# TariAgentBenchmark/unet-embroidery-seg

Hardware: AMD Instinct MI355X
Metric: images/sec training unet_resnet50 512×512 bf16 at 1/2/4/8 GPUs; mIoU parity (higher is better)
Workload: dtype bf16; 1 GPU; unet_resnet50 binary seg 512x512, per-GPU batch 16, lovasz_hinge + Adam; global_batch=16, image_size=512, parallelism=dp1

## Files before the change

### include/unetseg_hip.h

```cpp
#ifndef UNETSEG_HIP_H
#define UNETSEG_HIP_H

#include <stddef.h>
#include <stdint.h>

#ifdef __cplusplus
extern "C" {
#endif

const char* unetseg_last_error(void);
int unetseg_abi_version(void);
int unetseg_device_arch(char* buf, int n);


int unetseg_pack_conv_weight(int dtype, const float* w, int K, int C, int R, int S, int Cpad, void* wk, void* wt,
                             void* stream);
typedef struct UnetsegPackDesc {
  const float* w;
  void* wk;
  void* wt;
  long long start;
  int K, C, R, S, Cpad, Kld;
} UnetsegPackDesc;
int unetseg_pack_tiles(int K, int Cpad, int taps);
int unetseg_pack_conv_weights(int dtype, const void* desc, int n, long total, void* stream);
int unetseg_conv_tile_m(void);
int unetseg_conv2d_fwd_tile_m(int dtype, int c1, int ldc1, int c2, int ldc2, int n, int h, int w, int cout, int r,
                              int s, int stride, int pad);
int unetseg_conv2d_fwd(int dtype, const void* x1, int c1, int ldc1, const void* x2, int c2, int ldc2, int n, int h,
                       int w, const void* wk, int cout, int r, int s, int stride, int pad, const float* bias, int relu,
                       void* y, int ldy, float* stats, void* stream);
int unetseg_conv2d_fwd_bnrelu_in(int dtype, const void* x1, int c1, int ldc1, int n, int h, int w, const void* wk,
                                 int cout, const float* in_sc, const float* in_sh, const float* bias, int relu,
                                 void* y, int ldy, float* stats, void* stream);
int unetseg_conv2d_fwd_bnrelu_in_config(int dtype, int c1, int ldc1, int n, int h, int w, int cout);
int unetseg_conv2d_fwd_head_ok(int dtype, int ldc1, int n, int h, int w, int ldy, int head_k);
int unetseg_conv2d_fwd_head(int dtype, const void* x1, int ldc1, int n, int h, int w, const void* wk,
                            const float* bias, void* y, int ldy, int head_k, const float* head_w, const float* head_b,
                            float* logits, void* stream);
int unetseg_conv2d_fwd_mask(int dtype, const void* x1, int ldc1, int n, int h, int w, const void* wk,
                            const float* bias, void* y, int ldy, unsigned char* mbits, void* stream);
int unetseg_conv2d_wgrad_bnrelu_in(int dtype, const void* x1, int c1, int ldc1, int n, int h, int w, const void* dy,
                                   int ldy, int cout, const float* in_sc, const float* in_sh, float* ws,
                                   size_t ws_bytes, float* dw, int dw_c, int accumulate, void* stream);
int unetseg_conv2d_fwd_affine(int dtype, const void* x1, int c1, int ldc1, const void* x2, int c2, int ldc2, int n,
                              int h, int w, const void* wk, int cout, int r, int s, int stride, int pad,
                              const float* escale, const float* bias, int relu, void* y, int ldy, void* stream);
int unetseg_conv2d_fwd_config(int dtype, int c1, int ldc1, int c2, int ldc2, int n, int h, int w, int cout, int r,
                              int s, int stride, int pad, int* taps_out);
int unetseg_conv2d_dgrad_config(int dtype, int ldy, int n, int p, int q, int cout, int cin, int r, int s, int stride,
                                int pad, int ldx, int h, int w, int* cfg_out, int* taps_out);
int unetseg_conv2d_wgrad_config(int dtype, int c1, int ldc1, int c2, int ldc2, int n, int h, int w, int ldy, int cout,
                                int r, int s, int stride, int pad, int* splits_out);
int unetseg_conv2d_dgrad(int dtype, const void* dy, int ldy, int n, int p, int q, const void* wt, int cout, int cin,
                         int r, int s, int stride, int pad, void* dx, int ldx, int h, int w, int accumulate,
                         void* stream);
int unetseg_conv2d_dgrad_post(int dtype, const void* dy, int ldy, int n, int p, int q, const void* wt, int cout,
                              int cin, int r, int s, int stride, int pad, void* dx, int ldx, int h, int w, int post,
                              const void* aux, int ld_aux, const float* psc, const float* psh, const float* pmean,
                              const float* pinv, float* part, int rows, void* stream);
int unetseg_conv2d_dgrad_post_res(int dtype, const void* dy, int ldy, int n, int p, int q, const void* wt, int cout,
                                  int cin, void* dx, int ldx, const void* y1, int ld1, const float* mean1,
                                  const float* inv1, const unsigned char* mbits, const void* y2, int ld2,
                                  const float* mean2, const float* inv2, float* part, int rows, void* stream);
size_t unetseg_conv2d_wgrad_workspace(int dtype, int n, int p, int q, int cout, int cin, int r, int s);
int unetseg_conv2d_wgrad(int dtype, const void* x1, int c1, int ldc1, const void* x2, int c2, int ldc2, int n, int h,
                         int w, const void* dy, int ldy, int cout, int r, int s, int stride, int pad, float* ws,
                         size_t ws_bytes, float* dw, int dw_c, int accumulate, void* stream);
int unetseg_conv2d_wgrad_rows(int dtype, const void* x1, int c1, int ldc1, int n, int h, int w, const void* dy,
                              int ldy, int cout, int r, int s, int stride, int pad, float* ws, size_t ws_bytes,
                              float* dw, int dw_c, int accumulate, int dw_rows, void* stream);

int unetseg_pack_input_stem(const float* x, int n, int c, int h, int w, void* xp, void* stream);
int unetseg_stem_pack_weight(const float* w, int K, int C, void* wk, void* stream);
int unetseg_stem_fwd_tile_m(int n, int h, int w, int K);
int unetseg_stem_config(int n, int h, int w, int K, int* splits_out);
int unetseg_stem_fwd(const void* xp, int n, int h, int w, const void* wk, int K, void* y, int ldy, float* stats,
                     void* stream);
size_t unetseg_stem_wgrad_workspace(int n, int h, int w, int K);
int unetseg_stem_wgrad(const void* xp, int n, int h, int w, const void* dy, int ldy, int K, float* ws,
                       size_t ws_bytes, float* dw, int C, int accumulate, void* stream);
int unetseg_pack_input(int dtype, const float* x, int n, int c, int h, int w, int cpad, void* y, void* stream);


// ... 163 lines not shown
```

### unet-embroidery-seg_amd/csrc/conv.hip

```cpp
#include <cstdlib>

#include "common.h"
#include "conv_fast.h"

namespace {

constexpr int kBM = 128;

__device__ __forceinline__ int swz8(int row, int ch) { return ch ^ ((row >> 1) & 7); }
__device__ __forceinline__ int swz_tr(int row) { return ((row & 3) | ((row >> 1) & 4)) << 1; }

struct IgemmArgs {
  const void* x1;
  const void* x2;
  int c1, c2, ldc1, ldc2;
  int N, H, W;
  int hc, wc;
  int istride;
  int r0, rs, nr, dh0, dhs;
  int s0, ss, ns, dw0, dws;
  int S;
  int cin;
  const void* wt;
  long ldw;
// ... 1085 lines not shown
  if (k > 0) US_CHECK_ARG(launch_tn_multi(m, k, st) == 0, "conv2d_dgrad_post: merged launch refused");
  US_LAUNCH_CHECK("conv2d_dgrad_post");
  return 0;
}

UNETSEG_API int unetseg_conv2d_dgrad_post_res(int dtype, const void* dy, int ldy, int n, int p, int q, const void* wt,
                                              int cout, int cin, void* dx, int ldx, const void* y1, int ld1,
                                              const float* mean1, const float* inv1, const unsigned char* mbits,
                                              const void* y2, int ld2, const float* mean2, const float* inv2,
                                              float* part, int rows, void* stream) {
  if (dtype != DT_BF16 || n <= 0 || p <= 0 || q <= 0 || cout % 8 || ldy % 8 || cin % 8 || ldx < cin || ldx % 8)
    return 0;
  IgemmArgs a;
  if (!dgrad_classes(dy ? dy : kSomePtr, ldy, n, p, q, wt ? wt : kSomePtr, cout, cin, 1, 1, 1, 0,
                     dx ? dx : const_cast<void*>(kSomePtr), ldx, p, q, 0, 0, a) || a.M <= 0)
    return 0;
  FastTNArgs f;
  if (!fast_tn_args(a, f)) return 0;
  f.post = 3;
  f.accumulate = 0;
  if (!tn_fast_post_res_ok(f)) return 0;
  const int total = tn_fast_post_rows(f);
  if (!part) return total;
  US_CHECK_ARG(dy && wt && dx && y1 && mean1 && inv1 && mbits, "conv2d_dgrad_post_res: null pointer");
  US_CHECK_ARG(!y2 || (mean2 && inv2 && ld2 >= cin), "conv2d_dgrad_post_res: second branch needs y2, mean2, inv2");
  US_CHECK_ARG(ld1 >= cin, "conv2d_dgrad_post_res: ld1 < cin");
  US_CHECK_ARG(rows == total, "conv2d_dgrad_post_res: rows %d != %d", rows, total);
  f.aux = y1; f.ld_aux = ld1; f.pmean = mean1; f.pinv = inv1; f.mbits = mbits;
  f.aux2 = y2; f.ld_aux2 = ld2; f.pmean2 = mean2; f.pinv2 = inv2;
  f.ppart = part;
  US_CHECK_ARG(launch_tn_fast(f, (hipStream_t)stream) == 0, "conv2d_dgrad_post_res: no fused kernel");
  US_LAUNCH_CHECK("conv2d_dgrad_post_res");
  return 0;
}

UNETSEG_API int unetseg_conv2d_dgrad_config(int dtype, int ldy, int n, int p, int q, int cout, int cin, int r, int s,
                                            int stride, int pad, int ldx, int h, int w, int* cfg_out, int* taps_out) {
  US_CHECK_ARG(cfg_out && (stride == 1 || stride == 2), "conv2d_dgrad_config: bad args");
  int launched = 0;
  FastTNArgs fs[4];
  int idx[4], ncls = 0;
  bool fast = dtype == DT_BF16 && stride == 2;
  for (int ph = 0; ph < stride; ++ph)
    for (int pw = 0; pw < stride; ++pw) {
      const int k = ph * stride + pw;
      cfg_out[k] = -1;
      if (taps_out) taps_out[k] = 0;
      IgemmArgs a;
      if (!dgrad_classes(kSomePtr, ldy, n, p, q, kSomePtr, cout, cin, r, s, stride, pad, const_cast<void*>(kSomePtr), ldx, h, w, ph, pw, a))
        continue;
      if (a.M <= 0) continue;
      cfg_out[k] = tn_query(dtype, a, taps_out ? taps_out + k : nullptr);
      ++launched;
      if (fast) {
        idx[ncls] = k;
        fast = fast_tn_args(a, fs[ncls++]);
      }
    }
  bool in[4];
  const int bm = fast ? merge_plan(fs, ncls, in) : -1;
  if (bm > 0)
    for (int i = 0; i < ncls; ++i)
      if (in[i]) {
        cfg_out[idx[i]] = bm == 64 ? kCfgMulti64 : kCfgMulti128;
        if (taps_out) taps_out[idx[i]] = 0;
      }
// ... 314 lines not shown
```

### unet-embroidery-seg_amd/csrc/conv_fast.hip

```cpp
#include <cstdlib>
#include <type_traits>

#include "common.h"
#include "conv_fast.h"
#include "fast_util.h"


namespace {


template <int BM, int BN, int NWM, int NWN, int ST = 3>
constexpr int tn_waves_per_simd() {
  return ST == 5 ? (BN == 64 ? 4 : 3) : (BM == 64 || (BM == 128 && BN == 64)) ? 3 : 2;
}

template <int BM, int NWM, int NWN>
constexpr int kHaloChunks() {
  constexpr int NT = 64 * NWM * NWN;
  return ((BM / 32 + 2) * 34 * 8 + 2 * NT - 1) / (2 * NT) * (2 * NT);
}
template <int BM, int BN, int NWM, int NWN, int ST, int HA = 0>
constexpr size_t kPreOff() {
  constexpr size_t stages = HA ? ((size_t)2 * kHaloChunks<BM, NWM, NWN>() + (size_t)(ST - 10) * BN * 8) * 16
                               : (size_t)(ST == 1 || ST == 5 ? 1 : ST >= 13 ? ST - 10 : 2) * (BM + BN) * 8 * 16;
// ... 735 lines not shown
      float q = 0.f;
#pragma unroll
      for (int w = 0; w < NWM; ++w) {
        const float nw = (float)max(0, min(WTM, a.M - (m0 + w * WTM)));
        if (nw > 0.f) {
          const float d = red[w * BN + col] / nw - mean;
          q += red[(NWM + w) * BN + col] + nw * d * d;
        }
      }
      a.stats[(long)tile_m * 2 * a.Ng + n] = st;
      a.stats[(long)tile_m * 2 * a.Ng + a.Ng + n] = q;
    }
  }
}

template <int BM, int BN, int NWM, int NWN, int ST, int POST, int TAPS = 0, bool PRE = false, int HA = 0>
__global__ __launch_bounds__(64 * NWM * NWN, (tn_waves_per_simd<BM, BN, NWM, NWN, ST>())) void tn_fast_kernel(FastTNArgs a) {
  tn_fast_body<BM, BN, NWM, NWN, ST, POST, TAPS, PRE, HA>(a, blockIdx.x + gridDim.x * blockIdx.y, gridDim.x, gridDim.y);
}

struct TNMulti {
  FastTNArgs c[4];
  int start[5];
  int gx[4], gy[4];
  int n;
};

template <int BM, int BN, int NWM, int NWN, int ST, int POST>
__global__ __launch_bounds__(64 * NWM * NWN, (tn_waves_per_simd<BM, BN, NWM, NWN>())) void tn_multi_kernel(TNMulti m) {
  const int b = blockIdx.x;
  int k = 0;
  while (k + 1 < m.n && b >= m.start[k + 1]) ++k;
  tn_fast_body<BM, BN, NWM, NWN, ST, POST, 0, false>(m.c[k], b - m.start[k], m.gx[k], m.gy[k]);
}

template <int BN, int NWN>
constexpr size_t kPersistLds() {
  constexpr int HST = kHaloChunks<256, 4, NWN>();
  return (size_t)2 * HST * 16 + (size_t)3 * BN * 8 * 16 + (size_t)2 * 4 * BN * 4;
}

template <int BN, int NWN, int POST, int HA>
__global__ __launch_bounds__(512, 2) void tn_halo_persist_kernel(FastTNArgs a, int T, int ntiles, unsigned y_bytes) {
  constexpr int BM = 256, NWM = 4, NT = 512, NS = 3;
  constexpr int WTN = BN / NWN, FP = 4, FC = WTN / 16;
  constexpr int RSTEP = NT / 8;
  constexpr int B_PER = BN / RSTEP;
  static_assert(B_PER == 1 || B_PER == 2, "weight rows per thread");
  constexpr int HST = kHaloChunks<BM, NWM, NWN>();
  constexpr int HI = HST / NT;
  constexpr int HPIX = 10 * 34;
  constexpr int WST = BN * 8;
  constexpr int WP = B_PER;
  constexpr int HPC = HI / HA, TPER = 9 / HA;
  static_assert(HI % (2 * HA) == 0 && 9 % HA == 0, "halo pieces of whole instruction pairs");
  constexpr int NST = FC * FP;
  static_assert(WP + 2 * HPC + NST + 2 <= 63, "vmcnt range");
  extern __shared__ __attribute__((aligned(16))) uint4 lds[];

  const int tid = threadIdx.x, lane = tid & 63;
  const int wid = __builtin_amdgcn_readfirstlane(tid >> 6);
  const int wm = wid / NWN, wn = wid % NWN;
  const int kv = tid & 7, rb = tid >> 3;
  const int kg = lane >> 4, j16 = lane & 15;
  const int gy = (a.Ng + BN - 1) / BN;
  const int tpr = a.wc >> 5;
// ... 685 lines not shown
  const int min_t = m && atoi(m) > 0 ? atoi(m) : 2;
  const long T = (ntiles + (long)rounds * cu_count() - 1) / ((long)rounds * cu_count());
  return T >= min_t ? (int)T : 0;
}

template <int BN, int NWN, int HA>
static int launch_tn_persist(const FastTNArgs& a, hipStream_t st) {
  const int T = persist_t(a, BN);
  const size_t extra = (a.bias ? (size_t)a.Ng * 4 : 0) + (a.post == 2 ? (size_t)a.Ng * 16 : 0);
  const size_t lds = kPersistLds<BN, NWN>() + extra;
  const int ntiles = (a.M / 256) * ceil_div(a.Ng, BN);
  const int grid = ceil_div(ntiles, T);
  const unsigned y_bytes = (unsigned)((unsigned long long)a.M * (unsigned)a.ldy * 2ull);
  if (a.post) {
    static bool attr = false;
    if (!attr) {
      (void)hipFuncSetAttribute(reinterpret_cast<const void*>(&tn_halo_persist_kernel<BN, NWN, 1, HA>),
                                hipFuncAttributeMaxDynamicSharedMemorySize, 160 * 1024);
      attr = true;
    }
    hipLaunchKernelGGL((tn_halo_persist_kernel<BN, NWN, 1, HA>), dim3(grid), dim3(512), lds, st, a, T, ntiles, y_bytes);
  } else {
    static bool attr = false;
    if (!attr) {
      (void)hipFuncSetAttribute(reinterpret_cast<const void*>(&tn_halo_persist_kernel<BN, NWN, 0, HA>),
                                hipFuncAttributeMaxDynamicSharedMemorySize, 160 * 1024);
      attr = true;
    }
    hipLaunchKernelGGL((tn_halo_persist_kernel<BN, NWN, 0, HA>), dim3(grid), dim3(512), lds, st, a, T, ntiles, y_bytes);
  }
  return 0;
}

static int tn_config(const FastTNArgs& a) {
  if (a.force_cfg) return a.force_cfg;
  const int c = tn_config_base(a);
  if ((c == 7 || c == 13 || (c == 10 && !getenv("UNETSEG_TN_CFG_NO23"))) && halo_a_ok(a)) return c == 7 ? 21 : c == 13 ? 22 : 23;
  return c;
}

static int tn_config_base(const FastTNArgs& a) {
  if (const char* e = getenv("UNETSEG_TN_CFG")) {
    const int c = atoi(e);
    if (c == 21) return 7;
    if (((c >= 1 && c <= 14) || c == 19 || c == 20) && !(a.in_sc && c >= 7 && c <= 14)) return c;
  }
  static const bool no_dma_env = getenv("UNETSEG_TN_NO_DMA") != nullptr;
  const bool no_dma = no_dma_env || a.in_sc != nullptr;
  if (!a.in_sc && halo3_ok(a)) return 0;
  const int nsteps = a.nr * a.ns * (a.cin >> 6);
  static const bool no_short1 = getenv("UNETSEG_TN_NO_SHORT1") != nullptr;
  if (!no_short1 && nsteps <= 4 && (nsteps >= 2 || a.Ng <= 64)) return a.Ng <= 64 ? 20 : 19;
  if (nsteps == 1 && a.Ng > 64) return 4;
  if (a.Ng <= 64) return (!no_dma && nsteps >= 18 && tn_taps(a) == 9) ? 13 : 6;
  if (nsteps <= 4) return 3;
  const long tiles_big = (long)ceil_div(a.M, 256) * ceil_div(a.Ng, 128);
  if (tiles_big >= 256) return no_dma ? 2 : 7;
  const long tiles_mid = (long)ceil_div(a.M, 128) * ceil_div(a.Ng, 128);
  if (tiles_mid >= 256) return (!no_dma && nsteps >= 16 && tn_taps(a)) ? 10 : 3;
  return (!no_dma && nsteps >= 32) ? 9 : 5;
}

}

static int tn_cfg_bm(int cfg) {
  switch (cfg) {
    case 1: case 2: case 7: case 11: case 14: case 21: case 22: return 256;
    case 23: return 128;
    case 5: case 9: return 64;
    default: return 128;
  }
}

bool tn_fast_ok(const FastTNArgs& a) {
  return a.cin % 64 == 0 && a.c1 % 64 == 0 && a.nr * a.ns <= 32 && a.Ng % 8 == 0;
}

int tn_fast_tile_m(const FastTNArgs& a) {
  const int cfg = tn_config(a);
  return cfg == 0 ? halo_tile_m() : tn_cfg_bm(cfg);
}

int tn_fast_post_rows(const FastTNArgs& a) {
  if (a.M <= 0 || a.Ng <= 0) return 0;
  const int cfg = tn_config(a);
  return cfg == 0 ? halo3_blocks(a) : ceil_div(a.M, tn_cfg_bm(cfg));
}

int tn_fast_config(const FastTNArgs& a, int* taps_out) {
  const int cfg = tn_config(a);
  if ((cfg == 21 || cfg == 22) && !a.in_sc && a.post != 3 && a.post != 4 && persist_t(a, cfg == 21 ? 128 : 64) > 0) {
    if (taps_out) *taps_out = 0;
    return cfg + 3;
  }
  if (taps_out) *taps_out = (cfg >= 7 && cfg <= 14) ? tn_taps(a) : 0;
  return cfg;
}

bool tn_fast_post_res_ok(const FastTNArgs& a) {
  const int cfg = tn_config(a);
  return cfg == 4 || cfg == 19 || cfg == 20 || ((cfg == 7 || cfg == 10) && tn_taps(a) == 1);
}

static int launch_tn_post_res(const FastTNArgs& a, hipStream_t st) {
  switch (tn_config(a)) {
    case 4: return launch_tn_cfg<128, 128, 2, 2, 1, 3>(a, st);
    case 19: return launch_tn_cfg<128, 128, 2, 2, 5, 3>(a, st);
    case 20: return launch_tn_cfg<128, 64, 2, 2, 5, 3>(a, st);
    case 7: return tn_taps(a) == 1 ? launch_tn_cfg<256, 128, 4, 2, 13, 3, 1>(a, st) : -1;
    case 10: return tn_taps(a) == 1 ? launch_tn_cfg<128, 128, 2, 2, 15, 3, 1>(a, st) : -1;
    default: return -1;
  }
}

int launch_tn_fast(const FastTNArgs& a, hipStream_t st) {
  if (a.M <= 0 || a.Ng <= 0) return 0;
  if (a.post == 3) return a.in_sc ? -1 : launch_tn_post_res(a, st);
  if (a.post == 4) return tn_config(a) == 0 ? launch_halo3(a, st) : -1;
  if (a.in_sc) {
    switch (tn_config(a)) {
      case 1: return launch_tn_cfg<256, 64, 4, 1, 2, false, 0, true>(a, st);
      case 2: return launch_tn_cfg<256, 128, 4, 2, 3, false, 0, true>(a, st);
      case 4: return launch_tn_cfg<128, 128, 2, 2, 1, false, 0, true>(a, st);
      case 5: return launch_tn_cfg<64, 128, 1, 4, 3, false, 0, true>(a, st);
      case 6: return launch_tn_cfg<128, 64, 2, 2, 3, false, 0, true>(a, st);
      case 3: return launch_tn_cfg<128, 128, 2, 2, 3, false, 0, true>(a, st);
      case 19: return launch_tn_cfg<128, 128, 2, 2, 5, false, 0, true>(a, st);
      case 20: return launch_tn_cfg<128, 64, 2, 2, 5, false, 0, true>(a, st);
      default: return -1;
    }
  }
  switch (tn_config(a)) {
    case 0: return launch_halo3(a, st);
    case 1: return a.post ? launch_tn_cfg<256, 64, 4, 1, 2, true>(a, st) : launch_tn_cfg<256, 64, 4, 1, 2>(a, st);
    case 2: return a.post ? launch_tn_cfg<256, 128, 4, 2, 3, true>(a, st) : launch_tn_cfg<256, 128, 4, 2, 3>(a, st);
    case 4: return a.post ? launch_tn_cfg<128, 128, 2, 2, 1, true>(a, st) : launch_tn_cfg<128, 128, 2, 2, 1>(a, st);
    case 5: return a.post ? launch_tn_cfg<64, 128, 1, 4, 3, true>(a, st) : launch_tn_cfg<64, 128, 1, 4, 3>(a, st);
    case 6: return a.post ? launch_tn_cfg<128, 64, 2, 2, 3, true>(a, st) : launch_tn_cfg<128, 64, 2, 2, 3>(a, st);
    case 7: return launch_tn_dma<256, 128, 4, 2, 13>(a, st);
    case 8: return launch_tn_dma<128, 128, 2, 2, 14>(a, st);
    case 9: return launch_tn_dma<64, 128, 1, 4, 14>(a, st);
    case 10: return launch_tn_dma<128, 128, 2, 2, 15>(a, st);
    case 11: return launch_tn_dma<256, 64, 4, 1, 13>(a, st);
    case 12: return launch_tn_dma<128, 64, 2, 2, 14>(a, st);
    case 13: return launch_tn_dma<128, 64, 2, 2, 13>(a, st);
    case 14: return launch_tn_dma<256, 64, 4, 2, 13>(a, st);
    case 19: return a.post ? launch_tn_cfg<128, 128, 2, 2, 5, true>(a, st) : launch_tn_cfg<128, 128, 2, 2, 5>(a, st);
    case 20: return a.post ? launch_tn_cfg<128, 64, 2, 2, 5, true>(a, st) : launch_tn_cfg<128, 64, 2, 2, 5>(a, st);
    case 21: {
      if (persist_t(a, 128) > 0) return launch_tn_persist<128, 2, 3>(a, st);
      static const bool ns4 = getenv("UNETSEG_TN_HALO_NS4") != nullptr;
      static const bool split = !(getenv("UNETSEG_TN_HALO_SPLIT") && atoi(getenv("UNETSEG_TN_HALO_SPLIT")) == 1);
      if (ns4) return a.post ? launch_tn_cfg<256, 128, 4, 2, 14, true, 9, false, 1>(a, st)
                             : launch_tn_cfg<256, 128, 4, 2, 14, false, 9, false, 1>(a, st);
      if (split) return a.post ? launch_tn_cfg<256, 128, 4, 2, 13, true, 9, false, 3>(a, st)
                               : launch_tn_cfg<256, 128, 4, 2, 13, false, 9, false, 3>(a, st);
      return a.post ? launch_tn_cfg<256, 128, 4, 2, 13, true, 9, false, 1>(a, st)
                    : launch_tn_cfg<256, 128, 4, 2, 13, false, 9, false, 1>(a, st);
    }
    case 22:
      if (persist_t(a, 64) > 0) return launch_tn_persist<64, 2, 1>(a, st);
      return a.post ? launch_tn_cfg<256, 64, 4, 2, 13, true, 9, false, 1>(a, st)
                           : launch_tn_cfg<256, 64, 4, 2, 13, false, 9, false, 1>(a, st);
    case 23: return a.post ? launch_tn_cfg<128, 128, 2, 2, 15, true, 9, false, 1>(a, st)
                           : launch_tn_cfg<128, 128, 2, 2, 15, false, 9, false, 1>(a, st);
    default: return a.post ? launch_tn_cfg<128, 128, 2, 2, 3, true>(a, st) : launch_tn_cfg<128, 128, 2, 2, 3>(a, st);
  }
}

static bool tn_multi_off() {
  static const bool off = getenv("UNETSEG_NO_TN_MULTI") != nullptr;
  return off;
}

int tn_multi_tile_m(const FastTNArgs* fs, int n) {
  if (tn_multi_off() || n < 2 || n > 4) return -1;
  bool bm64 = false;
  for (int k = 0; k < n; ++k) {
    if (fs[k].in_sc || fs[k].M <= 0) return -1;
    const int cfg = tn_config(fs[k]);
    if (cfg == 0) return -1;
// ... 72 lines not shown
```

### unet-embroidery-seg_amd/unetseg_hip/introspect.py

```python
from __future__ import annotations

import os

from . import lib as _lib
from .lib import DT_BF16


def _out_hw(H, W, R, S, stride, pad):
    return (H + 2 * pad - R) // stride + 1, (W + 2 * pad - S) // stride + 1


def call_configs(desc, dt=DT_BF16):
    d, N, H, W, C1, C2, K, R, S, stride, pad, ld1, ld2 = desc
    cin = C1 + C2
    if d == "stem_fwd":
        cfg, _ = _lib.stem_config(N, H, W, K)
        return [f"stem_fwd:{cfg}"]
    if d == "stem_wgrad":
        Qs = (W - 1) // 2 + 1
        ring = Qs % 32 == 0 and not os.environ.get("UNETSEG_WG_NO_RING")
        tile = "wgrad64x256" if K <= 64 else "wgrad128"
        return [f"stem_wgrad:{'wgrad_ring64x256' if ring and K <= 64 else tile}", "reduce"]
    Pq, Qq = _out_hw(H, W, R, S, stride, pad)
    if d == "fwd":
        return ["fwd:" + _lib.fwd_config(dt, C1, ld1 or C1, C2, ld2 or C2, N, H, W, K, R, S, stride, pad)]
    if d == "fwd_affine":
        return ["fwd_affine:generic"]
    if d == "fwd_bnrelu_in":
        cfg = _lib.load().unetseg_conv2d_fwd_bnrelu_in_config(dt, C1, ld1 or C1, N, H, W, K)
        return ["fwd_bnrelu_in:" + _lib.CFG_NAMES.get(cfg, str(cfg))]
    if d in ("dgrad", "dgrad_post1", "dgrad_post2", "dgrad_post3", "dgrad_post4"):
        tag = "dgrad" if d == "dgrad" else d
        return [f"{tag}:{c}" for c in _lib.dgrad_config(dt, K, N, Pq, Qq, K, cin, R, S, stride, pad, cin, H, W)]
    if d == "dgrad_padk":
        Kp = -(-K // 64) * 64
        return [f"dgrad:{c}" for c in _lib.dgrad_config(dt, Kp, N, Pq, Qq, Kp, C1, 1, 1, 1, 0, C1, H, W)]
    if d == "wgrad_bnrelu_in":
        kern, sp, red = _lib.wgrad_config(dt, C1, ld1 or C1, 0, 0, N, H, W, K, K, 1, 1, 1, 0)
        return [f"wgrad_bnrelu_in:{kern}", red]
    if d in ("wgrad", "wgrad_padk"):
        Kw = -(-K // 64) * 64 if d == "wgrad_padk" else K
        c2 = 0 if d == "wgrad_padk" else C2
        kern, sp, red = _lib.wgrad_config(dt, C1, ld1 or C1, c2, ld2 or c2, N, H, W, Kw, Kw, R, S, stride, pad)
        return [f"wgrad:{kern}", red]
    raise ValueError(f"unknown probe direction {d!r}")


def probe_table(records, dt=DT_BF16):
    out = {}
    for kind, flops, nl, e0, e1, desc in records:
        t = e0.elapsed_time(e1) * 1e-3
        for i, key in enumerate(call_configs(desc, dt)):
            v = out.setdefault(key, [0, 0.0])
            v[0] += 1
            if i == 0:
                v[1] += t
    return out
```

### unet-embroidery-seg_amd/unetseg_hip/lib.py

```python
from __future__ import annotations

import ctypes
import os

_HERE = os.path.dirname(os.path.abspath(__file__))
LIB_PATH = os.environ.get("UNETSEG_LIB_PATH") or os.path.join(_HERE, "libunetseg_hip.so")

DT_F32, DT_BF16 = 0, 1

P = ctypes.c_void_p
I = ctypes.c_int
L = ctypes.c_long
F = ctypes.c_float
SZ = ctypes.c_size_t
ULL = ctypes.c_ulonglong
LL = ctypes.c_longlong

SIGNATURES = {
    "unetseg_last_error": (ctypes.c_char_p, []),
    "unetseg_abi_version": (I, []),
    "unetseg_device_arch": (I, [ctypes.c_char_p, I]),
    "unetseg_conv_tile_m": (I, []),
    "unetseg_conv2d_fwd": (I, [I, P, I, I, P, I, I, I, I, I, P, I, I, I, I, I, P, I, P, I, P, P]),
    "unetseg_conv2d_fwd_tile_m": (I, [I, I, I, I, I, I, I, I, I, I, I, I, I]),
# ... 41 lines not shown
    "unetseg_add": (I, [I, P, I, P, I, L, I, P]),
    "unetseg_lovasz_workspace": (SZ, [I, L]),
    "unetseg_lovasz_fwd": (I, [P, I, P, I, L, P, SZ, P, P, P]),
    "unetseg_bce_workspace": (SZ, [I, L]),
    "unetseg_bce_fwd": (I, [P, I, P, I, L, P, P, SZ, P, P, P]),
    "unetseg_dz_to_dout": (I, [P, I, L, I, P, F, P, F, P, P, P]),
    "unetseg_confusion": (I, [P, I, P, I, L, P, P]),
    "unetseg_adam": (I, [P, P, P, P, L, F, F, F, F, F, I, P, P]),
    "unetseg_gap_fwd": (I, [I, P, I, I, I, I, P, P]),
    "unetseg_gap_bwd": (I, [I, P, I, I, I, P, I, I, P]),
    "unetseg_linear_fwd": (I, [P, P, P, I, I, I, I, F, ULL, P, P, P, P, P]),
    "unetseg_linear_bwd": (I, [P, P, P, F, I, P, P, I, I, I, P, P, P, P, P]),
    "unetseg_ce_fwd": (I, [P, P, I, I, P, P, P]),
    "unetseg_scale_grad": (I, [P, L, P, F, P, F, P, P]),
    "unetseg_stream_wait": (I, [P, P]),
    "unetseg_stream_create_cumask": (I, [P, I, P]),
    "unetseg_conv2d_dgrad_post": (I, [I, P, I, I, I, I, P, I, I, I, I, I, I, P, I, I, I, I, P, I, P, P, P, P, P, I,
                                      P]),
    "unetseg_bn_bwd_finalize_rows": (I, [P, I, I, L, P, P, P, P, P, P]),
    "unetseg_fin_merge_rows": (I, [P, I, I, L, I, I, P, P]),
    "unetseg_conv2d_dgrad_post_res": (I, [I, P, I, I, I, I, P, I, I, P, I, P, I, P, P, P, P, I, P, P, P, I, P]),
    "unetseg_bn_bwd_finalize_rows_res": (I, [P, I, I, L, I, P, P, P, P, P, P, P, P, P, P]),
    "unetseg_colsum_rows": (I, [P, I, I, I, P, I, P]),
    "unetseg_pack_input_stem": (I, [P, I, I, I, I, P, P]),
    "unetseg_stem_pack_weight": (I, [P, I, I, P, P]),
    "unetseg_stem_fwd_tile_m": (I, [I, I, I, I]),
    "unetseg_stem_fwd": (I, [P, I, I, I, P, I, P, I, P, P]),
    "unetseg_stem_wgrad_workspace": (SZ, [I, I, I, I]),
    "unetseg_stem_wgrad": (I, [P, I, I, I, P, I, I, P, SZ, P, I, I, P]),
    "unetseg_adam_dev": (I, [P, P, P, P, L, P, P, F, F, F, F, P, P]),
    "unetseg_conv2d_fwd_config": (I, [I, I, I, I, I, I, I, I, I, I, I, I, I, P]),
    "unetseg_conv2d_dgrad_config": (I, [I, I, I, I, I, I, I, I, I, I, I, I, I, I, P, P]),
    "unetseg_conv2d_wgrad_config": (I, [I, I, I, I, I, I, I, I, I, I, I, I, I, I, P]),
    "unetseg_stem_config": (I, [I, I, I, I, P]),
    "unetseg_pw_head_fwd": (I, [I, P, I, L, I, I, I, P, P, P, P]),
    "unetseg_pw_head_tiles": (I, [L]),
    "unetseg_pw_head_bwd": (I, [I, P, P, I, L, I, I, I, P, P, I, I, P, P, P]),
    "unetseg_mc_loss_workspace": (SZ, [I, I, L]),
    "unetseg_mc_loss_fwd": (I, [P, P, I, I, L, P, L, I, F, F, P, I, F, F, P, SZ, P, P]),
    "unetseg_mc_loss_bwd": (I, [P, P, I, I, L, P, L, I, F, F, P, I, F, F, P, P, P, P]),
    "unetseg_mc_confusion": (I, [P, P, I, I, L, P, P]),
    "unetseg_softmax_resize_argmax": (I, [P, I, I, I, I, I, I, I, I, I, P, P]),
    "unetseg_resize_bilinear_fwd": (I, [I, P, I, I, I, I, I, I, I, I, P, I, P]),
    "unetseg_resize_bilinear_bwd": (I, [I, P, I, I, I, I, I, I, I, I, P, I, I, P]),
    "unetseg_pad2d_fwd": (I, [I, P, I, I, I, I, I, I, I, I, I, P, I, P]),
    "unetseg_pad2d_bwd": (I, [I, P, I, I, I, I, I, I, I, I, I, P, I, I, P]),
    "unetseg_confusion_masked": (I, [P, I, P, I, L, L, P, P]),
    "unetseg_masked_loss_workspace": (SZ, [I, L]),
    "unetseg_masked_loss_fwd": (I, [P, I, P, I, L, L, I, P, P, SZ, P, P, P]),
    "unetseg_lovasz_fwd_masked": (I, [P, I, P, I, L, L, P, SZ, P, P, P]),
    "unetseg_channel_stats_tiles": (I, [L, I]),
    "unetseg_channel_stats": (I, [I, P, I, L, I, I, P, P]),
    "unetseg_augment_tables_len": (I, [LL, LL, LL, LL, LL]),
    "unetseg_augment_batch": (I, [P, P, I, P, P, LL, P, LL, P, LL, P, LL, P, LL, I, I, I, I, P, P, P, P]),
    "unetseg_augment_batch_dev": (I, [P, P, I, P, P, LL, P, LL, P, LL, P, LL, P, LL, I, I, I, I, P, P, P, P]),
    "unetseg_augment_tables_dev": (I, [P, I, P, P, I, P]),
    "unetseg_tile_count": (I, [I, I, I, I, P, P]),
    "unetseg_tile_gather": (I, [P, I, I, I, I, I, I, I, P, P]),
    "unetseg_tile_accum": (I, [P, I, I, I, I, I, I, I, P, P]),
    "unetseg_tile_finish": (I, [P, I, I, I, I, I, P, P, P]),
}

VALUE_FUNCS = {"conv2d_fwd_mask", "reduce_tiles", "pw_small_tiles", "conv_tile_m", "abi_version", "conv2d_fwd_tile_m",
               "conv2d_dgrad_post", "conv2d_dgrad_post_res", "stem_fwd_tile_m", "attn_bwd1_tiles", "pw_small_tile", "conv2d_fwd_config",
               "conv2d_dgrad_config", "conv2d_wgrad_config", "stem_config", "pw_head_tiles", "channel_stats_tiles",
               "augment_tables_len", "pack_tiles",
               "conv2d_fwd_bnrelu_in_config", "conv2d_fwd_head_ok", "upsample2x_bwd_tiles"}

_lib = None


class HipUnavailable(RuntimeError):
    pass


def load(path: str = LIB_PATH):
    global _lib
    if _lib is not None:
        return _lib
    if not os.path.exists(path):
        raise HipUnavailable(
            f"libunetseg_hip.so not found at {path}: build it with `python -c 'import __graft_entry__ as g; g.build()'` "
            "(hipcc --offload-arch=gfx950).  There is no CPU fallback.")
    lib = ctypes.CDLL(path)
    for name, (res, args) in SIGNATURES.items():
        fn = getattr(lib, name)
        fn.restype = res
        fn.argtypes = args
    _lib = lib
    return lib


def exported_symbols():
    return list(SIGNATURES)


def last_error() -> str:
    return load().unetseg_last_error().decode("utf-8", "replace")
# ... 29 lines not shown
_WRAP = None


class _Caller:

    def __getattr__(self, item):
        lib_ = load()
        fast = _fast()
        if fast is not None and hasattr(fast, item):
            fn = getattr(fast, item)
        else:
            raw = getattr(lib_, "unetseg_" + item)
            if SIGNATURES["unetseg_" + item][0] is I and item not in VALUE_FUNCS:
                def fn(*args, _raw=raw):
                    rc = _raw(*args)
                    if rc != 0:
                        raise RuntimeError(f"unetseg_{item} failed ({rc}): {last_error()}")
                    return rc
            else:
                fn = raw
        if _WRAP is not None:
            return _WRAP(item, fn)
        self.__dict__[item] = fn
        return fn


lib = _Caller()


CFG_NAMES = {0: "halo3", 1: "tn256x64", 2: "tn256x128", 3: "tn128x128", 4: "tn128x128_1step", 5: "tn64x128",
             6: "tn128x64", 7: "ring256x128", 8: "ring128x128", 9: "ring64x128", 10: "ring128x128_5st",
             11: "ring256x64", 12: "ring128x64_4st", 13: "ring128x64", 14: "ring256x64_8w", 17: "multi128x128",
             18: "multi64x128", 19: "tn128x128_1st", 20: "tn128x64_1st", 21: "ring256x128_halo", 22: "ring256x64_halo",
             23: "ring128x128_halo", 24: "ring256x128_hp", 25: "ring256x64_hp", 30: "stem_halo", 31: "first3x3", 100: "generic"}
WG_NAMES = {0: "halo3_wgrad", 1: "wgrad64x256_row", 2: "wgrad128_row", 3: "wgrad64x256", 4: "wgrad128",
            5: "wgrad_generic", 6: "wgrad_ring64x256", 7: "wgrad_ring128"}


def _cfg_name(cfg, taps):
    n = CFG_NAMES.get(cfg, str(cfg))
    return f"{n}_t{taps}" if taps else n


def fwd_config(dtype, c1, ldc1, c2, ldc2, n, h, w, cout, r, s, stride, pad):
    taps = ctypes.c_int(0)
    cfg = load().unetseg_conv2d_fwd_config(dtype, c1, ldc1, c2, ldc2, n, h, w, cout, r, s, stride, pad,
                                           ctypes.byref(taps))
    return _cfg_name(cfg, taps.value)


def dgrad_config(dtype, ldy, n, p, q, cout, cin, r, s, stride, pad, ldx, h, w):
    cfg = (ctypes.c_int * 4)()
    taps = (ctypes.c_int * 4)()
    load().unetseg_conv2d_dgrad_config(dtype, ldy, n, p, q, cout, cin, r, s, stride, pad, ldx, h, w, cfg, taps)
    return [_cfg_name(cfg[i], taps[i]) for i in range(stride * stride) if cfg[i] >= 0]


def wgrad_config(dtype, c1, ldc1, c2, ldc2, n, h, w, ldy, cout, r, s, stride, pad):
    sp = ctypes.c_int(0)
    kind = load().unetseg_conv2d_wgrad_config(dtype, c1, ldc1, c2, ldc2, n, h, w, ldy, cout, r, s, stride, pad,
                                              ctypes.byref(sp))
    return WG_NAMES.get(kind, str(kind)), sp.value, "reduce"


def tile_count(h, w, tile, overlap):
    nx, ny = ctypes.c_int(0), ctypes.c_int(0)
    lib.tile_count(h, w, tile, overlap, ctypes.addressof(nx), ctypes.addressof(ny))
# ... 8 lines not shown
```

Measured before the change: 1050 images/s.

## Add persistent panel kernel for 1x1 dgrad keeping activation panel resident in LDS

Adds a new 1x1 data-gradient GEMM kernel. Each workgroup loads a full 128-row panel of dy across all input channels (up to 256) into LDS once, then sweeps the weight tiles over output columns, so the A operand is not reloaded for every N tile. It is selected by default only for the accumulate case without a post-op, and behind an environment flag for the fused residual post case. It trades LDS capacity (up to 5 stages) and simple single-buffered weight staging with barriers for the saved activation reloads.

```diff
diff --git a/include/unetseg_hip.h b/include/unetseg_hip.h
--- a/include/unetseg_hip.h
+++ b/include/unetseg_hip.h
@@ -50,6 +50,8 @@
                               int s, int stride, int pad, int* taps_out);
 int unetseg_conv2d_dgrad_config(int dtype, int ldy, int n, int p, int q, int cout, int cin, int r, int s, int stride,
                                 int pad, int ldx, int h, int w, int* cfg_out, int* taps_out);
+int unetseg_conv2d_dgrad_1x1_config(int dtype, int ldy, int n, int p, int q, int cout, int cin, int ldx, int post,
+                                    int accumulate);
 int unetseg_conv2d_wgrad_config(int dtype, int c1, int ldc1, int c2, int ldc2, int n, int h, int w, int ldy, int cout,
                                 int r, int s, int stride, int pad, int* splits_out);
 int unetseg_conv2d_dgrad(int dtype, const void* dy, int ldy, int n, int p, int q, const void* wt, int cout, int cin,
diff --git a/unet-embroidery-seg_amd/csrc/conv.hip b/unet-embroidery-seg_amd/csrc/conv.hip
--- a/unet-embroidery-seg_amd/csrc/conv.hip
+++ b/unet-embroidery-seg_amd/csrc/conv.hip
@@ -1141,6 +1141,19 @@
   US_CHECK_ARG(launch_tn_fast(f, (hipStream_t)stream) == 0, "conv2d_dgrad_post_res: no fused kernel");
   US_LAUNCH_CHECK("conv2d_dgrad_post_res");
   return 0;
+}
+
+UNETSEG_API int unetseg_conv2d_dgrad_1x1_config(int dtype, int ldy, int n, int p, int q, int cout, int cin, int ldx,
+                                                int post, int accumulate) {
+  IgemmArgs a;
+  if (!dgrad_classes(kSomePtr, ldy, n, p, q, kSomePtr, cout, cin, 1, 1, 1, 0, const_cast<void*>(kSomePtr), ldx, p, q, 0,
+                     0, a) || a.M <= 0)
+    return -1;
+  FastTNArgs f;
+  if (dtype != DT_BF16 || !fast_tn_args(a, f)) return kCfgGeneric;
+  f.post = post == 3 ? 3 : 0;
+  f.accumulate = post == 3 ? 0 : accumulate;
+  return tn_fast_config(f, nullptr);
 }
 
 UNETSEG_API int unetseg_conv2d_dgrad_config(int dtype, int ldy, int n, int p, int q, int cout, int cin, int r, int s,
diff --git a/unet-embroidery-seg_amd/csrc/conv_fast.hip b/unet-embroidery-seg_amd/csrc/conv_fast.hip
--- a/unet-embroidery-seg_amd/csrc/conv_fast.hip
+++ b/unet-embroidery-seg_amd/csrc/conv_fast.hip
@@ -791,6 +791,248 @@
   int k = 0;
   while (k + 1 < m.n && b >= m.start[k + 1]) ++k;
   tn_fast_body<BM, BN, NWM, NWN, ST, POST, 0, false>(m.c[k], b - m.start[k], m.gx[k], m.gy[k]);
+}
+
+constexpr int kPanelStage = 128 * 128;
+
+template <int POST, bool ACC>
+__global__ __launch_bounds__(256, 2) void tn_panel_kernel(FastTNArgs a, int npanels, int nsplit, int gy) {
+  constexpr int BM = 128, BN = 128, NWM = 2, NWN = 2, NT = 256;
+  constexpr int WTM = 64, WTN = 64, FP = 4, FC = 4;
+  constexpr int RSTEP = NT / 8, A_PER = BM / RSTEP, B_PER = BN / RSTEP;
+  constexpr int MAXCH = 4;
+  extern __shared__ __attribute__((aligned(16))) uint4 lds[];
+  const int tid = threadIdx.x, lane = tid & 63;
+  const int wid = __builtin_amdgcn_readfirstlane(tid >> 6);
+  const int wm = wid / NWN, wn = wid % NWN;
+  const int kv = tid & 7, rb = tid >> 3;
+  const int nch = a.cin >> 6;
+  uint4* const wst = lds + nch * (kPanelStage / 16);
+  const __amdgpu_buffer_rsrc_t r1 = srd(a.x1, a.x1_bytes);
+  const __amdgpu_buffer_rsrc_t rw = srd(a.wt, a.w_bytes);
+
+  unsigned foffA[2], foffB[2];
+#pragma unroll
+  for (int kk = 0; kk < 2; ++kk) {
+    const int r = lane & 15, sw = ((kk * 4 + (lane >> 4)) ^ ((r >> 1) & 7)) * 16;
+    foffA[kk] = (unsigned)((wm * WTM + r) * 128 + sw);
+    foffB[kk] = (unsigned)((wn * WTN + r) * 128 + sw);
+  }
+  auto wload = [&](uint4 (&rbv)[B_PER], int tn, int s) {
+#pragma unroll
+    for (int i = 0; i < B_PER; ++i) {
+      const int n = tn * BN + rb + RSTEP * i;
+      rbv[i] = bload(rw, n < a.Ng ? (unsigned)n * (unsigned)a.ldwb + (unsigned)(s * 128 + kv * 16) : kOOB);
+    }
+  };
+  auto wstore = [&](const uint4 (&rbv)[B_PER]) {
+#pragma unroll
+    for (int i = 0; i < B_PER; ++i) {
+      const int row = rb + RSTEP * i;
+      wst[row * 8 + swz8(row, kv)] = rbv[i];
+    }
+  };
+
+  const int kg = lane >> 4, j16 = lane & 15;
+  constexpr int LROW = WTN * 2 + 16;
+  char* const tl = reinterpret_cast<char*>(wst) + wid * (16 * LROW);
+  float* const red = reinterpret_cast<float*>(reinterpret_cast<char*>(wst) + NWM * NWN * 16 * LROW);
+  constexpr int CPR = WTN / 8, RPI = 64 / CPR, NIT = WTM / RPI;
+  constexpr int GRP = POST == 3 ? 2 : 4;
+  static_assert(RPI == 8 && NIT == 8, "two 8-row store instructions per 16-row transpose");
+  const int ck = lane % CPR, rsub = lane / CPR;
+  const bool two = POST == 3 && a.aux2 != nullptr;
+  constexpr bool kOps = POST == 3 || ACC;
+
+  const int items = npanels * nsplit;
+#pragma unroll 1
+  for (int item = blockIdx.x; item < items; item += gridDim.x) {
+    const int panel = item / nsplit, part = item - panel * nsplit;
+    const int t0 = part * gy / nsplit, t1 = (part + 1) * gy / nsplit;
+    const int m0 = panel * BM;
+    uint4 wreg[B_PER];
+    {
+      uint4 ra[MAXCH][A_PER];
+#pragma unroll
+      for (int s = 0; s < MAXCH; ++s)
+        if (s < nch) {
+#pragma unroll
+          for (int i = 0; i < A_PER; ++i) {
+            const int m = m0 + rb + RSTEP * i;
+            ra[s][i] = bload(r1, m < a.M ? (unsigned)m * (unsigned)a.ldc1b + (unsigned)(s * 128 + kv * 16) : kOOB);
+          }
+        }
+      wload(wreg, t0, 0);
+      __syncthreads();
+#pragma unroll
+      for (int s = 0; s < MAXCH; ++s)
+        if (s < nch) {
+#pragma unroll
+          for (int i = 0; i < A_PER; ++i) {
+            const int row = rb + RSTEP * i;
+            lds[s * (kPanelStage / 16) + row * 8 + swz8(row, kv)] = ra[s][i];
+          }
+        }
+    }
+    const int row0 = m0 + wm * WTM;
+    const int cnt = min(WTM, a.M - row0);
+
+#pragma unroll 1
+    for (int tn = t0; tn < t1; ++tn) {
+      const int n0 = tn * BN;
+      const int nc = n0 + wn * WTN + ck * 8;
+      const int ncl = nc < a.Ng ? nc : a.Ng - 8;
+      const bf16* aux2p = two ? (const bf16*)a.aux2 : (const bf16*)a.aux;
+      const long ld2 = two ? a.ld_aux2 : a.ld_aux;
+      uint4 oldv[kOps ? NIT : 1], zv[POST == 3 ? NIT : 1], z2v[POST == 3 ? NIT : 1];
+      unsigned mkv[POST == 3 ? NIT : 1];
+      auto opload = [&](int it) {
+        const int r = it * RPI + rsub;
+        const long opx = r < cnt ? row0 + r : min(row0, a.M - 1);
+        oldv[it] = *reinterpret_cast<const uint4*>((const bf16*)a.y + opx * a.ldy + ncl);
+        if constexpr (POST == 3) {
+          zv[it] = *reinterpret_cast<const uint4*>((const bf16*)a.aux + opx * a.ld_aux + ncl);
+          z2v[it] = *reinterpret_cast<const uint4*>(aux2p + opx * ld2 + ncl);
+          mkv[it] = (unsigned)a.mbits[opx * (a.Ng >> 3) + (ncl >> 3)];
+        }
+      };
+      if constexpr (kOps) {
+#pragma unroll
+        for (int it = 0; it < GRP; ++it) opload(it);
+      }
+
+      f32x4 acc[FC][FP];
+#pragma unroll
+      for (int c = 0; c < FC; ++c)
+#pragma unroll
+        for (int p = 0; p < FP; ++p) acc[c][p] = f32x4{0.f, 0.f, 0.f, 0.f};
+#pragma unroll 1
+      for (int kt = 0; kt < nch; ++kt) {
+        __syncthreads();
+        wstore(wreg);
+        __syncthreads();
+        const bool last = kt + 1 == nch;
+        if (!last || tn + 1 < t1) wload(wreg, last ? tn + 1 : tn, last ? 0 : kt + 1);
+        const char* sa = reinterpret_cast<const char*>(lds + kt * (kPanelStage / 16));
+        const char* sb = reinterpret_cast<const char*>(wst);
+#pragma unroll
+        for (int kk = 0; kk < 2; ++kk) {
+          bf16x8 pf[FP], wf[FC];
+#pragma unroll
+          for (int p = 0; p < FP; ++p) pf[p] = *reinterpret_cast<const bf16x8*>(sa + foffA[kk] + p * 2048);
+#pragma unroll
+          for (int c = 0; c < FC; ++c) wf[c] = *reinterpret_cast<const bf16x8*>(sb + foffB[kk] + c * 2048);
+#pragma unroll
+          for (int c = 0; c < FC; ++c)
+#pragma unroll
+            for (int p = 0; p < FP; ++p)
+              acc[c][p] = __builtin_amdgcn_mfma_f32_16x16x32_bf16(wf[c], pf[p], acc[c][p], 0, 0, 0);
+        }
+      }
+      __syncthreads();
+
+      constexpr int NQ3 = POST == 3 ? 8 : 1;
+      float q3[3][NQ3], mu3[2][NQ3], iv3[2][NQ3];
+      if constexpr (POST == 3) {
+#pragma unroll
+        for (int e = 0; e < 8; ++e) {
+          const bool ok = nc + e < a.Ng;
+          q3[0][e] = q3[1][e] = q3[2][e] = 0.f;
+          mu3[0][e] = ok ? a.pmean[nc + e] : 0.f;
+          iv3[0][e] = ok ? a.pinv[nc + e] : 0.f;
+          mu3[1][e] = (ok && two) ? a.pmean2[nc + e] : 0.f;
+          iv3[1][e] = (ok && two) ? a.pinv2[nc + e] : 0.f;
+        }
+      }
+#pragma unroll
+      for (int p = 0; p < FP; ++p) {
+        const bool mok = p * 16 + j16 < cnt;
+#pragma unroll
+        for (int c = 0; c < FC; ++c) {
+          bf16 ob[4];
+#pragma unroll
+          for (int e = 0; e < 4; ++e) {
+            const float v = acc[c][p][e] + 0.f;
+            ob[e] = (bf16)(mok ? (float)(bf16)v : 0.f);
+          }
+          *reinterpret_cast<uint2*>(tl + j16 * LROW + (c * 16 + kg * 4) * 2) = *reinterpret_cast<uint2*>(ob);
+        }
+        __builtin_amdgcn_s_waitcnt(0xC07F);
+        __builtin_amdgcn_wave_barrier();
+#pragma unroll
+        for (int i2 = 0; i2 < 2; ++i2) {
+          const int it = p * 2 + i2;
+          const int r = it * RPI + rsub;
+          uint4 v = *reinterpret_cast<const uint4*>(tl + (i2 * RPI + rsub) * LROW + ck * 16);
+          if (r >= cnt || nc >= a.Ng) continue;
+          bf16* ptr = (bf16*)a.y + (long)(row0 + r) * a.ldy + nc;
+          if constexpr (POST == 3) {
+            const uint4 old = oldv[it], z = zv[it], z2 = z2v[it];
+            const unsigned mk = mkv[it];
+            const bf16* ob = reinterpret_cast<const bf16*>(&old);
+            const bf16* zb = reinterpret_cast<const bf16*>(&z);
+            const bf16* z2b = reinterpret_cast<const bf16*>(&z2);
+            bf16* nv = reinterpret_cast<bf16*>(&v);
+#pragma unroll
+            for (int e = 0; e < 8; ++e) {
+              const bf16 sm = (bf16)((float)nv[e] + (float)ob[e]);
+              const float d = ((mk >> e) & 1u) ? (float)sm : 0.f;
+              nv[e] = (bf16)d;
+              q3[0][e] += d;
+              q3[1][e] = fmaf(d, ((float)zb[e] - mu3[0][e]) * iv3[0][e], q3[1][e]);
+              if (two) q3[2][e] = fmaf(d, ((float)z2b[e] - mu3[1][e]) * iv3[1][e], q3[2][e]);
+            }
+          } else if constexpr (ACC) {
+            const uint4 old = oldv[it];
+            const bf16* ob = reinterpret_cast<const bf16*>(&old);
+            bf16* nv = reinterpret_cast<bf16*>(&v);
+#pragma unroll
+            for (int e = 0; e < 8; ++e) nv[e] = (bf16)((float)nv[e] + (float)ob[e]);
+          }
+          *reinterpret_cast<uint4*>(ptr) = v;
+        }
+        __builtin_amdgcn_wave_barrier();
+        if constexpr (kOps) {
+          if (2 * p + GRP < NIT) {
+            opload(2 * p + GRP);
+            opload(2 * p + GRP + 1);
+          }
+        }
+      }
+      if constexpr (POST == 3) {
+#pragma unroll
+        for (int q = 0; q < 3; ++q)
+#pragma unroll
+          for (int e = 0; e < 8; ++e)
+            for (int o = CPR; o < 64; o <<= 1) q3[q][e] += __shfl_xor(q3[q][e], o, 64);
+        if (rsub == 0) {
+#pragma unroll
+          for (int e = 0; e < 8; ++e) {
+            const int col = wn * WTN + ck * 8 + e;
+            red[wm * BN + col] = q3[0][e];
+            red[(NWM + wm) * BN + col] = q3[1][e];
+            red[(2 * NWM + wm) * BN + col] = q3[2][e];
+          }
+        }
+        const int nq = a.aux2 ? 3 : 2;
+        asm volatile("s_waitcnt lgkmcnt(0)\n\ts_barrier" ::: "memory");
+        for (int col = tid; col < BN; col += NT) {
+          const int n = n0 + col;
+          if (n >= a.Ng) continue;
+          float s0 = 0.f, s1 = 0.f, s2 = 0.f;
+#pragma unroll
+          for (int w = 0; w < NWM; ++w) {
+            s0 += red[w * BN + col];
+            s1 += red[(NWM + w) * BN + col];
+            s2 += red[(2 * NWM + w) * BN + col];
+          }
+          a.ppart[(long)panel * nq * a.Ng + n] = s0;
+          a.ppart[(long)panel * nq * a.Ng + a.Ng + n] = s1;
+          if (nq == 3) a.ppart[(long)panel * nq * a.Ng + 2 * a.Ng + n] = s2;
+        }
+      }
+    }
+  }
 }
 
 template <int BN, int NWN>
@@ -1542,9 +1784,57 @@
   return 0;
 }
 
+static bool panel_ok(const FastTNArgs& a) {
+  if (a.nr != 1 || a.ns != 1 || a.dh0 || a.dw0 || a.r0 || a.s0 || a.istride != 1) return false;
+  if (a.ostride != 1 || a.ph || a.pw || a.OH != a.hc || a.OW != a.wc || a.H != a.hc || a.W != a.wc) return false;
+  if (a.x2 || a.c1 != a.cin || a.cin % 64 || a.cin > 256 || a.Ng <= 64 || a.Ng % 8) return false;
+  if (a.in_sc || a.bias || a.relu || a.stats || a.head_w || a.mbits_out || a.t2d) return false;
+  return a.post == 0 || (a.post == 3 && !a.accumulate);
+}
+static bool panel_on(const FastTNArgs& a) {
+  const char* e = getenv("UNETSEG_TN_PANEL");
+  const int mode = e ? atoi(e) : 1;
+  if (mode <= 0 || !panel_ok(a)) return false;
+  return mode >= 2 || (a.post == 0 && a.accumulate);
+}
+static int env_pos(const char* name) {
+  const char* e = getenv(name);
+  return e && atoi(e) > 0 ? atoi(e) : 0;
+}
+static int launch_tn_panel(const FastTNArgs& a, hipStream_t st) {
+  const int nch = a.cin >> 6;
+  const size_t lds = (size_t)(nch + 1) * kPanelStage;
+  const int npanels = ceil_div(a.M, 128), gy = ceil_div(a.Ng, 128);
+  const int slots = 2 * cu_count();
+  int nsplit = env_pos("UNETSEG_TN_PANEL_SPLIT");
+  if (!nsplit)
+    for (nsplit = 1; nsplit < gy && (long)npanels * nsplit < slots; ++nsplit) {}
+  if (nsplit > gy) nsplit = gy;
+  const long items = (long)npanels * nsplit;
+  int grid = env_pos("UNETSEG_TN_PANEL_GRID");
+  if (!grid) grid = slots;
+  if (grid > items) grid = (int)items;
+#define PANEL_LAUNCH(POST, ACC)                                                                                      \
+  do {                                                                                                               \
+    static bool attr = false;                                                                                        \
+    if (!attr) {                                                                                                     \
+      (void)hipFuncSetAttribute(reinterpret_cast<const void*>(&tn_panel_kernel<POST, ACC>),                          \
+                                hipFuncAttributeMaxDynamicSharedMemorySize, 5 * kPanelStage);                        \
+      attr = true;                                                                                                   \
+    }                                                                                                                \
+    hipLaunchKernelGGL((tn_panel_kernel<POST, ACC>), dim3(grid), dim3(256), lds, st, a, npanels, nsplit, gy);        \
+  } while (0)
+  if (a.post == 3) PANEL_LAUNCH(3, false);
+  else if (a.accumulate) PANEL_LAUNCH(0, true);
+  else PANEL_LAUNCH(0, false);
+#undef PANEL_LAUNCH
+  return 0;
+}
+
 static int tn_config(const FastTNArgs& a) {
   if (a.force_cfg) return a.force_cfg;
   const int c = tn_config_base(a);
+  if ((c == 19 || c == 4) && panel_on(a)) return 26;
   if ((c == 7 || c == 13 || (c == 10 && !getenv("UNETSEG_TN_CFG_NO23"))) && halo_a_ok(a)) return c == 7 ? 21 : c == 13 ? 22 : 23;
   return c;
 }
@@ -1609,7 +1899,7 @@
 
 bool tn_fast_post_res_ok(const FastTNArgs& a) {
   const int cfg = tn_config(a);
-  return cfg == 4 || cfg == 19 || cfg == 20 || ((cfg == 7 || cfg == 10) && tn_taps(a) == 1);
+  return cfg == 4 || cfg == 19 || cfg == 20 || cfg == 26 || ((cfg == 7 || cfg == 10) && tn_taps(a) == 1);
 }
 
 static int launch_tn_post_res(const FastTNArgs& a, hipStream_t st) {
@@ -1617,6 +1907,7 @@
     case 4: return launch_tn_cfg<128, 128, 2, 2, 1, 3>(a, st);
     case 19: return launch_tn_cfg<128, 128, 2, 2, 5, 3>(a, st);
     case 20: return launch_tn_cfg<128, 64, 2, 2, 5, 3>(a, st);
+    case 26: return launch_tn_panel(a, st);
     case 7: return tn_taps(a) == 1 ? launch_tn_cfg<256, 128, 4, 2, 13, 3, 1>(a, st) : -1;
     case 10: return tn_taps(a) == 1 ? launch_tn_cfg<128, 128, 2, 2, 15, 3, 1>(a, st) : -1;
     default: return -1;
@@ -1657,6 +1948,7 @@
     case 14: return launch_tn_dma<256, 64, 4, 2, 13>(a, st);
     case 19: return a.post ? launch_tn_cfg<128, 128, 2, 2, 5, true>(a, st) : launch_tn_cfg<128, 128, 2, 2, 5>(a, st);
     case 20: return a.post ? launch_tn_cfg<128, 64, 2, 2, 5, true>(a, st) : launch_tn_cfg<128, 64, 2, 2, 5>(a, st);
+    case 26: return launch_tn_panel(a, st);
     case 21: {
       if (persist_t(a, 128) > 0) return launch_tn_persist<128, 2, 3>(a, st);
       static const bool ns4 = getenv("UNETSEG_TN_HALO_NS4") != nullptr;
diff --git a/unet-embroidery-seg_amd/unetseg_hip/introspect.py b/unet-embroidery-seg_amd/unetseg_hip/introspect.py
--- a/unet-embroidery-seg_amd/unetseg_hip/introspect.py
+++ b/unet-embroidery-seg_amd/unetseg_hip/introspect.py
@@ -31,6 +31,9 @@
         return ["fwd_bnrelu_in:" + _lib.CFG_NAMES.get(cfg, str(cfg))]
     if d in ("dgrad", "dgrad_post1", "dgrad_post2", "dgrad_post3", "dgrad_post4"):
         tag = "dgrad" if d == "dgrad" else d
+        if d == "dgrad_post3":
+            cfg = _lib.load().unetseg_conv2d_dgrad_1x1_config(dt, K, N, Pq, Qq, K, cin, cin, 3, 0)
+            return [f"{tag}:" + _lib.CFG_NAMES.get(cfg, str(cfg))]
         return [f"{tag}:{c}" for c in _lib.dgrad_config(dt, K, N, Pq, Qq, K, cin, R, S, stride, pad, cin, H, W)]
     if d == "dgrad_padk":
         Kp = -(-K // 64) * 64
diff --git a/unet-embroidery-seg_amd/unetseg_hip/lib.py b/unet-embroidery-seg_amd/unetseg_hip/lib.py
--- a/unet-embroidery-seg_amd/unetseg_hip/lib.py
+++ b/unet-embroidery-seg_amd/unetseg_hip/lib.py
@@ -97,6 +97,7 @@
     "unetseg_conv2d_fwd_config": (I, [I, I, I, I, I, I, I, I, I, I, I, I, I, P]),
     "unetseg_conv2d_dgrad_config": (I, [I, I, I, I, I, I, I, I, I, I, I, I, I, I, P, P]),
     "unetseg_conv2d_wgrad_config": (I, [I, I, I, I, I, I, I, I, I, I, I, I, I, I, P]),
+    "unetseg_conv2d_dgrad_1x1_config": (I, [I, I, I, I, I, I, I, I, I, I]),
     "unetseg_stem_config": (I, [I, I, I, I, P]),
     "unetseg_pw_head_fwd": (I, [I, P, I, L, I, I, I, P, P, P, P]),
     "unetseg_pw_head_tiles": (I, [L]),
@@ -128,7 +129,7 @@
 
 VALUE_FUNCS = {"conv2d_fwd_mask", "reduce_tiles", "pw_small_tiles", "conv_tile_m", "abi_version", "conv2d_fwd_tile_m",
                "conv2d_dgrad_post", "conv2d_dgrad_post_res", "stem_fwd_tile_m", "attn_bwd1_tiles", "pw_small_tile", "conv2d_fwd_config",
-               "conv2d_dgrad_config", "conv2d_wgrad_config", "stem_config", "pw_head_tiles", "channel_stats_tiles",
+               "conv2d_dgrad_config", "conv2d_dgrad_1x1_config", "conv2d_wgrad_config", "stem_config", "pw_head_tiles", "channel_stats_tiles",
                "augment_tables_len", "pack_tiles",
                "conv2d_fwd_bnrelu_in_config", "conv2d_fwd_head_ok", "upsample2x_bwd_tiles"}
 
@@ -224,7 +225,7 @@
              6: "tn128x64", 7: "ring256x128", 8: "ring128x128", 9: "ring64x128", 10: "ring128x128_5st",
              11: "ring256x64", 12: "ring128x64_4st", 13: "ring128x64", 14: "ring256x64_8w", 17: "multi128x128",
              18: "multi64x128", 19: "tn128x128_1st", 20: "tn128x64_1st", 21: "ring256x128_halo", 22: "ring256x64_halo",
-             23: "ring128x128_halo", 24: "ring256x128_hp", 25: "ring256x64_hp", 30: "stem_halo", 31: "first3x3", 100: "generic"}
+             23: "ring128x128_halo", 24: "ring256x128_hp", 25: "ring256x64_hp", 26: "panel128", 30: "stem_halo", 31: "first3x3", 100: "generic"}
 WG_NAMES = {0: "halo3_wgrad", 1: "wgrad64x256_row", 2: "wgrad128_row", 3: "wgrad64x256", 4: "wgrad128",
             5: "wgrad_generic", 6: "wgrad_ring64x256", 7: "wgrad_ring128"}
 
```

New measurement: 1050 images/s (median of 2 runs). Within noise of the previous version (-0.0%).
